# stateless-consensus/phant

Measured on AMD Instinct MI355X. Metric: mpt_proofs_verified_per_sec_depth8, higher is better.
Workload: dtype u64; 1 GPU; config3: 100000 synthetic depth-8 account proofs per GPU against one state root (7 x 532 B full branches + 112 B leaf, 3868 B and 29 Keccak-f per proof, 1% corrupted/exclusion, no cross-proof dedup); every launch sequence in flight verifies its own witness (seeds 2..3: distinct data per slot), 30 back-to-back passes per timed step; parallelism=key-sharded x1, verify_mode=flat, streams=2

## Files before the change

### phant_amd/csrc/mpt_verify_v3.hip

```cpp
#include <phant_platform.h>

#include "launch.h"
#include "mpt_verify_one.hip.h"
#include "coop_sponge.hip.h"
#include "verify_hash.hip.h"

namespace phant {
namespace v3 {
using namespace vh;

constexpr uint32_t HDR_PFN_BROKEN = 9;
constexpr uint32_t HDR_SLOW = 10;
constexpr uint32_t HDR_OPENED = 11;
constexpr uint32_t HDR_PARITY = 15;
constexpr uint32_t HDR_STAT = 1024;
constexpr uint32_t HDR_STAT_STRIPES = 16;
constexpr uint32_t HDR_STAT_WORDS = HDR_STAT_STRIPES * N_CLASS;
constexpr uint32_t HDR_STAT_END = HDR_STAT + 2u * HDR_STAT_WORDS;
constexpr uint32_t HDR_CUR = 256;
constexpr uint32_t HDR_WORDS = 768;
constexpr size_t HEADER_BYTES = 8192;
static_assert(HDR_STAT_END <= VERIFY_HEADER_WORDS && 4u * VERIFY_HEADER_WORDS <= HEADER_BYTES,
              "capi.hip copies VERIFY_HEADER_WORDS words back for the statistics");

PHANT_DEV uint32_t cursor_word(uint32_t cls, uint32_t stripe) { return HDR_CUR + 32u * stripe + cls; }



PHANT_DEV uint64_t key_prefix64(const uint8_t* __restrict__ key, uint32_t key_len) {
    uint64_t kb = 0;
    const uint32_t take = key_len < 8u ? key_len : 8u;
    for (uint32_t t = 0; t < take; ++t) kb |= (uint64_t)key[t] << (56u - 8u * t);
    return kb;
}
PHANT_DEV uint64_t key_prefix64_wide(const uint8_t* __restrict__ key, uint32_t key_len) {
    if (key_len < 8u) return key_prefix64(key, key_len);
    struct __attribute__((packed, aligned(1))) U64u { unsigned long long v; };
    return __builtin_bswap64(reinterpret_cast<const U64u*>(key)->v);
}
PHANT_DEV bool same_prefix(uint64_t x, uint64_t y, uint32_t d) { return d == 0u || ((x ^ y) >> (64u - 4u * d)) == 0ull; }
PHANT_DEV uint64_t group_hash(uint64_t kb, uint32_t root, uint32_t d) {
    const uint64_t pre = d ? (kb >> (64u - 4u * d)) : 0ull;
    uint64_t h = pre ^ ((uint64_t)(d + 1u) << 58) ^ ((uint64_t)root * 0x9E3779B97F4A7C15ull);
    h ^= h >> 33;
    h *= 0xff51afd7ed558ccdull;
    h ^= h >> 33;
    h *= 0xc4ceb9fe1a85ec53ull;
    h ^= h >> 33;
    return h;
}
PHANT_DEV uint32_t direct_index(uint64_t kb, uint32_t root, uint32_t d, uint32_t n_roots) {
    uint32_t width = 1u, below = 0u;
    for (uint32_t t = 0; t < d; ++t) {
        below += width;
        width <<= 4;
    }
    const uint32_t pre = d ? (uint32_t)(kb >> (64u - 4u * d)) : 0u;
    return n_roots * below + root * width + pre;
}
PHANT_DEV uint32_t slot_a(uint64_t h, uint32_t mask) { return (uint32_t)h & mask; }
PHANT_DEV uint32_t slot_b(uint64_t h, uint32_t mask) { return (uint32_t)(h >> 24) & mask; }

struct Args {
    VerifyArgs v;
    uint32_t total_nodes;
    uint32_t shallow;
    uint32_t direct;
    uint32_t* dtab;
    uint64_t* table;
    uint32_t tmask;
    uint32_t* rep;
    uint2* ent;
    uint32_t stripe_cap;
    uint32_t* hdr;
    uint32_t* digest;
    uint8_t* nstat;
};

PHANT_DEV void beside_the_hashing() { __builtin_amdgcn_s_setprio(3); }

__global__ void __launch_bounds__(256) zero_kernel(uint4* p, size_t n16, uint32_t* fail_count, uint32_t n_roots) {
    beside_the_hashing();
    const size_t i = (size_t)blockIdx.x * 256u + threadIdx.x;
    if (i < n16) p[i] = make_uint4(0u, 0u, 0u, 0u);
    if (fail_count)
        for (size_t r = i; r < n_roots; r += (size_t)gridDim.x * 256u) fail_count[r] = 0u;
}

struct ShallowLane {
    uint32_t p, d, j, root, len;
    uint64_t kb;
    bool act;
    bool valid;
    bool group;
    bool broken;
};
PHANT_DEV ShallowLane shallow_node(const Args& a, uint32_t p, uint32_t d) {
    ShallowLane L;
    L.p = p;
    L.d = d;
    L.j = 0;
    L.root = 0;
    L.len = 0;
    L.kb = 0;
    L.act = L.valid = L.group = L.broken = false;
    if (L.p >= a.v.n) return L;
    const uint32_t first = a.v.proof_first_node[L.p], last = a.v.proof_first_node[L.p + 1];
    if (last < first) {
        L.broken = L.d == 0u;
        return L;
    }
    if (last > a.total_nodes) return L;
    const uint32_t nn = 2u * a.v.key_len, cnt = last - first;
    const uint32_t end = cnt <= nn ? cnt : nn + 1u;
    if (L.d >= end) return L;
    L.act = true;
    L.j = first + L.d;
    L.root = a.v.root_idx ? a.v.root_idx[L.p] : 0u;
    const uint64_t e = a.v.node_off[L.j + 1], b = a.v.node_off[L.j];
    if (e >= b && e <= a.v.nodes_len && e - b <= 0x7fffffffull) {
        L.valid = true;
        L.len = (uint32_t)(e - b);
    }
    L.group = L.valid && L.len >= RATE && L.root < a.v.n_roots;
    if (L.group) L.kb = key_prefix64(a.v.keys + (uint64_t)a.v.key_len * L.p, a.v.key_len);
    return L;
}
PHANT_DEV ShallowLane shallow_lane(const Args& a, uint32_t g) {
    const uint32_t p = g / a.shallow;
    return shallow_node(a, p, g - p * a.shallow);
}

PHANT_DEV void clear_launch_state(const Args& a, uint32_t g, size_t lanes) {
    const uint32_t other = HDR_STAT + HDR_STAT_WORDS * ((a.hdr[HDR_PARITY] & 1u) ^ 1u);
    for (size_t i = g; i < HDR_WORDS + HDR_STAT_WORDS; i += lanes) {
        if (i < HDR_WORDS) {
            if (i != HDR_PARITY) a.hdr[i] = 0u;
        } else {
            a.hdr[other + (i - HDR_WORDS)] = 0u;
        }
    }
    if (a.v.fail_count)
        for (size_t r = g; r < a.v.n_roots; r += lanes) a.v.fail_count[r] = 0u;
}

__global__ void __launch_bounds__(256) propose_kernel(const Args a) {
    beside_the_hashing();
    const uint32_t g = blockIdx.x * 256u + threadIdx.x;
    clear_launch_state(a, g, (size_t)gridDim.x * 256u);
    const ShallowLane L = shallow_lane(a, g);
    if (L.act) a.nstat[L.j] = 0u;
    if (!L.group) return;
    if (L.d < a.direct) {
        a.dtab[direct_index(L.kb, L.root, L.d, a.v.n_roots)] = L.j + 1u;
    } else {
        const uint64_t h = group_hash(L.kb, L.root, L.d);
        const uint64_t entry = ((uint64_t)L.p << 32) | (uint64_t)(L.j + 1u);
        a.table[slot_a(h, a.tmask)] = entry;
        a.table[slot_b(h, a.tmask)] = entry;
    }
}

PHANT_DEV bool entry_matches(const Args& a, uint64_t en, const ShallowLane& L, uint32_t& node) {
    const uint32_t pr = (uint32_t)(en >> 32), j1 = (uint32_t)en;
    if (j1 == 0u || pr >= a.v.n) return false;
    node = j1 - 1u;
    if (pr == L.p) return node == L.j;
    const uint32_t f = a.v.proof_first_node[pr], l = a.v.proof_first_node[pr + 1];
    if (l < f || l > a.total_nodes || node < f || node >= l || node - f != L.d) return false;
    if ((a.v.root_idx ? a.v.root_idx[pr] : 0u) != L.root) return false;
    return same_prefix(key_prefix64(a.v.keys + (uint64_t)a.v.key_len * pr, a.v.key_len), L.kb, L.d);
}

PHANT_DEV uint64_t ent_index(const Args& a, uint32_t cls, uint32_t stripe, uint32_t at) {
    return ((uint64_t)cls * STRIPES + stripe) * a.stripe_cap + at;
}

PHANT_DEV bool wave_bytes_equal(const uint8_t* x, const uint8_t* y, uint32_t len, uint32_t lane) {
    uint32_t diff = 0;
    const uint32_t full = len & ~15u;
    for (uint32_t o = 16u * lane; o < full; o += 1024u) {
        const uint4 p = load16u(x + o), q = load16u(y + o);
        diff |= (p.x ^ q.x) | (p.y ^ q.y) | (p.z ^ q.z) | (p.w ^ q.w);
    }
    if (lane < (len & 15u)) diff |= (uint32_t)(x[full + lane] ^ y[full + lane]);
    return __ballot(diff != 0) == 0ull;
}

constexpr int COMPARE_UNROLL = 4;

__global__ void __launch_bounds__(256) PHANT_NUM_VGPR(48) dedup_kernel(const Args a) {
    constexpr uint32_t WAVES = 4;
    __shared__ uint32_t s_cnt[WAVES][N_LIST];
    __shared__ uint32_t s_base[N_LIST];
    beside_the_hashing();
    const uint32_t tid = threadIdx.x, lane = tid & 63u, wave = tid >> 6;
    const uint32_t NT = a.total_nodes;
    if (tid < WAVES * N_LIST) (&s_cnt[0][0])[tid] = 0u;
    const ShallowLane L = shallow_lane(a, blockIdx.x * 256u + tid);
    if (L.broken) a.hdr[HDR_PFN_BROKEN] = 1u;

    const uint32_t j = L.j;
    uint32_t cand = j;
    uint64_t b = 0, cb = 0;
    if (L.group) {
        uint32_t c = j;
        if (L.d < a.direct) {
            const uint32_t t = a.dtab[direct_index(L.kb, L.root, L.d, a.v.n_roots)];
            if (t) c = t - 1u;
        } else {
            const uint64_t h = group_hash(L.kb, L.root, L.d);
            uint32_t node;
            if (entry_matches(a, a.table[slot_a(h, a.tmask)], L, node)) c = node;
            else if (entry_matches(a, a.table[slot_b(h, a.tmask)], L, node)) c = node;
        }
        if (c != j && c < NT) {
            const uint64_t c0 = a.v.node_off[c], c1 = a.v.node_off[c + 1];
            if (c1 >= c0 && c1 <= a.v.nodes_len && c1 - c0 == L.len) {
                cand = c;
                cb = c0;
                b = a.v.node_off[j];
            }
        }
    }

    const uint32_t coff = 16u * (lane & 31u);
    const bool upper = lane >= 32u;
    const uint32_t b_lo = (uint32_t)b, b_hi = (uint32_t)(b >> 32), cb_lo = (uint32_t)cb, cb_hi = (uint32_t)(cb >> 32);
    bool differs = false;
    const bool is532 = cand != j && L.len == BRANCH_LEN;
    unsigned long long todo = __ballot(is532);
    while (todo) {
        uint32_t i0[COMPARE_UNROLL], i1[COMPARE_UNROLL];
        uint4 x[COMPARE_UNROLL], y[COMPARE_UNROLL];
        uint32_t i = 0;
#pragma unroll
        for (int u = 0; u < COMPARE_UNROLL; ++u) {
            if (todo) {
                i = (uint32_t)__builtin_ctzll(todo);
                todo &= todo - 1ull;
            }
            i0[u] = i;
            if (todo) {
                i = (uint32_t)__builtin_ctzll(todo);
                todo &= todo - 1ull;
            }
            i1[u] = i;
            const uint64_t own0 = lane_u64(b_lo, b_hi, i0[u]), own1 = lane_u64(b_lo, b_hi, i1[u]);
            const uint64_t oth0 = lane_u64(cb_lo, cb_hi, i0[u]), oth1 = lane_u64(cb_lo, cb_hi, i1[u]);
            x[u] = load16u(a.v.nodes + (upper ? own1 : own0) + coff);
            y[u] = load16u(a.v.nodes + (upper ? oth1 : oth0) + coff);
        }
#pragma unroll
        for (int u = 0; u < COMPARE_UNROLL; ++u) {
            uint32_t diff = x[u].x ^ y[u].x;
            diff = __builtin_amdgcn_bitop3_b32(x[u].y, y[u].y, diff, 0xBE);
            diff = __builtin_amdgcn_bitop3_b32(x[u].z, y[u].z, diff, 0xBE);
            diff = __builtin_amdgcn_bitop3_b32(x[u].w, y[u].w, diff, 0xBE);
            const unsigned long long m = __ballot(diff != 0);
            if ((uint32_t)m != 0u && lane == i0[u]) differs = true;
            if ((uint32_t)(m >> 32) != 0u && lane == i1[u]) differs = true;
        }
    }
    if (is532 && !differs) {
        const uint8_t* const own = a.v.nodes + b + (BRANCH_LEN - 28u);
        const uint8_t* const oth = a.v.nodes + cb + (BRANCH_LEN - 28u);
        const uint4 p0 = load16u(own), p1 = load16u(own + 12), q0 = load16u(oth), q1 = load16u(oth + 12);
        uint32_t diff = (p0.x ^ q0.x) | (p0.y ^ q0.y) | (p0.z ^ q0.z) | (p0.w ^ q0.w);
        diff |= (p1.x ^ q1.x) | (p1.y ^ q1.y) | (p1.z ^ q1.z) | (p1.w ^ q1.w);
        if (diff) differs = true;
    }
    todo = __ballot(cand != j && L.len != BRANCH_LEN);
    while (todo) {
        const uint32_t i = (uint32_t)__builtin_ctzll(todo);
        todo &= todo - 1ull;
        const uint32_t ll = lane_u32(L.len, i);
        const bool eq = wave_bytes_equal(a.v.nodes + lane_u64(b_lo, b_hi, i), a.v.nodes + lane_u64(cb_lo, cb_hi, i), ll, lane);
        if (lane == i && !eq) differs = true;
    }
    if (differs) cand = j;
    if (L.act) a.rep[j] = cand;

    const uint32_t cls = (L.act && L.valid && cand == j) ? node_list(L.len) : CLASS_NONE;
    uint32_t my_rank = 0;
    __syncthreads();
    todo = __ballot(cls != CLASS_NONE);
    while (todo) {
        const uint32_t c0 = lane_u32(cls, (uint32_t)__builtin_ctzll(todo));
        const unsigned long long m = __ballot(cls == c0);
        if (lane == 0) s_cnt[wave][c0] = (uint32_t)__popcll(m);
        if (cls == c0) my_rank = (uint32_t)__popcll(m & ((1ull << lane) - 1ull));
        todo &= ~m;
    }
    __syncthreads();
    const uint32_t stripe = blockIdx.x % STRIPES;
    if (tid < N_LIST) {
        uint32_t tot = 0;
        for (uint32_t w = 0; w < WAVES; ++w) tot += s_cnt[w][tid];
        s_base[tid] = tot ? atomicAdd(&a.hdr[cursor_word(tid, stripe)], tot) : 0u;
    }
    __syncthreads();
    if (cls != CLASS_NONE) {
        uint32_t at = s_base[cls] + my_rank;
        for (uint32_t w = 0; w < wave; ++w) at += s_cnt[w][cls];
        a.ent[ent_index(a, cls, stripe, at)] = make_uint2(j, L.p);
    }
}


PHANT_DEV const uint8_t* ref_location(const Args& a, uint32_t j, uint32_t d, uint32_t root, uint32_t nib_parent, uint64_t b) {
    if (d == 0u) return root < a.v.n_roots ? a.v.roots + 32ull * root : nullptr;
    if (nib_parent >= 16u) return nullptr;
    const uint64_t pb = a.v.node_off[j - 1u];
    if (pb > b || b - pb != BRANCH_LEN) return nullptr;
    return a.v.nodes + pb + (4u + 33u * nib_parent);
}

struct RefBytes { uint4 lo, hi; };
PHANT_DEV RefBytes load_ref(const uint8_t* q) {
    RefBytes r;
    r.lo = r.hi = make_uint4(0, 0, 0, 0);
    if (q) {
        r.lo = load16u(q);
        r.hi = load16u(q + 16);
    }
    return r;
}
PHANT_DEV bool digest_equals(const Sponge& s, const RefBytes& r) {
    const uint32_t diff = (s.lo[0] ^ r.lo.x) | (s.hi[0] ^ r.lo.y) | (s.lo[1] ^ r.lo.z) | (s.hi[1] ^ r.lo.w) |
                          (s.lo[2] ^ r.hi.x) | (s.hi[2] ^ r.hi.y) | (s.lo[3] ^ r.hi.z) | (s.hi[3] ^ r.hi.w);
    return diff == 0u;
}
PHANT_DEV void store_node_digest(const Args& a, uint32_t j, const Sponge& s) {
    uint4* o = reinterpret_cast<uint4*>(a.digest + 8ull * j);
    o[0] = make_uint4(s.lo[0], s.hi[0], s.lo[1], s.hi[1]);
    o[1] = make_uint4(s.lo[2], s.hi[2], s.lo[3], s.hi[3]);
}


PHANT_DEV bool list_role(const Args& a, uint32_t q, const uint32_t lane) {
    static_assert(N_QUEUE > 64u && N_QUEUE <= 128u, "two lists per lane");
    const uint32_t cnt_a = a.hdr[cursor_word(queue_class(lane), lane % STRIPES)];
    const uint32_t cnt_b = lane + 64u < N_QUEUE ? a.hdr[cursor_word(queue_class(lane + 64u), (lane + 64u) % STRIPES)] : 0u;
    const uint32_t ch_a = (cnt_a + 63u) / 64u, ch_b = (cnt_b + 63u) / 64u;
    const uint32_t incl_a = wave_inclusive_scan(ch_a, lane);
    uint32_t li, before, cnt;
    const unsigned long long m_a = __ballot(q < incl_a);
    if (m_a) {
        const uint32_t l = (uint32_t)__builtin_ctzll(m_a);
        li = l;
        before = lane_u32(incl_a, l) - lane_u32(ch_a, l);
        cnt = lane_u32(cnt_a, l);
    } else {
        const uint32_t incl_b = lane_u32(incl_a, 63u) + wave_inclusive_scan(ch_b, lane);
        const unsigned long long m_b = __ballot(q < incl_b);
        if (!m_b) return false;
        const uint32_t l = (uint32_t)__builtin_ctzll(m_b);
        li = l + 64u;
        before = lane_u32(incl_b, l) - lane_u32(ch_b, l);
        cnt = lane_u32(cnt_b, l);
    }
    const uint32_t cls = queue_class(li), stripe = li % STRIPES;
    uint32_t idx = (q - before) * 64u + lane;
    idx = idx < cnt ? idx : cnt - 1u;
    const uint2 en = a.ent[ent_index(a, cls, stripe, idx)];
    const uint32_t j = en.x;
    const uint8_t* const safe_end = a.v.nodes + a.v.nodes_len;
    const uint64_t b = a.v.node_off[j];
    const uint32_t len = (uint32_t)(a.v.node_off[j + 1] - b);
    const uint8_t* const p = a.v.nodes + b;

    const uint8_t* refp = nullptr;
    {
        const uint32_t owner = en.y;
        const uint32_t d = j - a.v.proof_first_node[owner];
        const uint32_t root = a.v.root_idx ? a.v.root_idx[owner] : 0u;
        uint32_t nibp = 16u;
        if (d >= 1u && d - 1u < 2u * a.v.key_len) nibp = key_nibble(a.v.keys + (uint64_t)a.v.key_len * owner, d - 1u);
        refp = ref_location(a, j, d, root, nibp, b);
    }
    const RefBytes ref = load_ref(refp);

    Sponge s;
    uint32_t bad;
    const uint32_t len0 = (uint32_t)__builtin_amdgcn_readfirstlane(len);
    if (cls == LIST_B532) {
        bad = hash_b532<true>(s, p);
    } else if (cls == 0u && __ballot(len != len0 || p + RATE > safe_end) == 0ull) {
        hash_short_uniform(s, p, len0);
        bad = 1u;
    } else {
        hash_any(s, p, len, safe_end);
        bad = 1u;
    }
    uint32_t ns = NS_HASHED | (bad == 0u ? NS_CANON : 0u);
    if (refp) ns |= NS_LINK_CHECKED | (digest_equals(s, ref) ? NS_LINK_OK : 0u);
    a.nstat[j] = (uint8_t)ns;
    store_node_digest(a, j, s);
    return true;
}

constexpr uint32_t DEEP_LEVELS = 8;

template <bool SOLO>
PHANT_DEV void deep_role(const Args& a, const uint32_t w, const uint32_t lane, const uint32_t waves_per_level, const uint32_t levels,
                         uint32_t (&s_ref)[8][256]) {
    const uint32_t level = w / waves_per_level;
    if (level >= levels) return;
    const uint32_t p = (w % waves_per_level) * 64u + lane;
    const uint8_t* const safe_end = a.v.nodes + a.v.nodes_len;
    const uint32_t nn = 2u * a.v.key_len;
    uint32_t hashed[N_CLASS] = {0, 0, 0, 0, 0, 0, 0, 0};
    const uint32_t stat_buf = a.hdr[HDR_PARITY] & 1u;
    for (uint32_t d = a.shallow + level;; d += levels) {
        uint32_t first = 0, count = 0, root = 0;
        if (p < a.v.n) {
            first = a.v.proof_first_node[p];
            const uint32_t last = a.v.proof_first_node[p + 1];
            if (last >= first && last <= a.total_nodes) count = last - first;
            if constexpr (SOLO) {
                if (last < first) a.hdr[HDR_PFN_BROKEN] = 1u;
            }
            if (a.v.root_idx) root = a.v.root_idx[p];
        }
        if (__ballot(d < count) == 0ull) break;
        const uint32_t j = first + d;
        bool active = d < count;
        uint64_t b = 0;
        uint32_t len = 0;
        if (active) {
            const uint64_t e = a.v.node_off[j + 1];
            b = a.v.node_off[j];
            active = e >= b && e <= a.v.nodes_len && e - b <= 0x7fffffffull;
            len = active ? (uint32_t)(e - b) : 0u;
            if (!active) a.nstat[j] = 0u;
        }
        const bool roomy = a.v.nodes_len >= BRANCH_LEN;
        const uint8_t* const ptr = a.v.nodes + (active ? b : 0ull);
        const uint8_t* refp = nullptr;
        if (active) {
            const uint8_t* const key = a.v.keys + (uint64_t)a.v.key_len * p;
            const uint32_t nibp = (d >= 1u && d - 1u < nn) ? key_nibble(key, d - 1u) : 16u;
            refp = ref_location(a, j, d, root, nibp, b);
        }
        {
            const RefBytes ref = load_ref(refp);
            const uint32_t t = threadIdx.x;
            s_ref[0][t] = ref.lo.x; s_ref[1][t] = ref.lo.y; s_ref[2][t] = ref.lo.z; s_ref[3][t] = ref.lo.w;
            s_ref[4][t] = ref.hi.x; s_ref[5][t] = ref.hi.y; s_ref[6][t] = ref.hi.z; s_ref[7][t] = ref.hi.w;
        }
        {
            const uint32_t cls = len / RATE < N_CLASS ? len / RATE : N_CLASS - 1u;
#pragma unroll
            for (uint32_t c = 0; c < N_CLASS; ++c) hashed[c] += (uint32_t)__popcll(__ballot(active && cls == c));
        }
        enum : uint32_t { F_ACTIVE = 1u, F_REF = 2u, F_CANON = 4u };
        uint32_t flags = (active ? F_ACTIVE : 0u) | (refp != nullptr ? F_REF : 0u);
        Sponge s;
        const bool is532 = active && len == BRANCH_LEN;
        if (roomy && __ballot(is532) != 0ull) {
            const uint32_t bad = hash_b532<true>(s, is532 ? ptr : a.v.nodes);
            if (is532 && bad == 0u) flags |= F_CANON;
        }
        const bool rest = active && !(roomy && is532);
        if (__ballot(rest) != 0ull) {
            const uint32_t len0 = (uint32_t)__builtin_amdgcn_readfirstlane(len);
            if (len0 < RATE && __ballot(!rest || len != len0 || ptr + RATE > safe_end) == 0ull) {
                hash_short_uniform(s, ptr, len0);
            } else if (rest) {
                hash_any(s, ptr, len, safe_end);
            }
        }
        if (flags & F_ACTIVE) {
            const uint32_t j = a.v.proof_first_node[p] + d;
            uint32_t ns = NS_HASHED | ((flags & F_CANON) ? NS_CANON : 0u);
            if (flags & F_REF) {
                const uint32_t t = threadIdx.x;
                RefBytes ref;
                ref.lo = make_uint4(s_ref[0][t], s_ref[1][t], s_ref[2][t], s_ref[3][t]);
                ref.hi = make_uint4(s_ref[4][t], s_ref[5][t], s_ref[6][t], s_ref[7][t]);
                ns |= NS_LINK_CHECKED | (digest_equals(s, ref) ? NS_LINK_OK : 0u);
            }
            a.nstat[j] = (uint8_t)ns;
            store_node_digest(a, j, s);
        }
    }
    if (lane < N_CLASS) {
        uint32_t mine = 0;
#pragma unroll
        for (uint32_t c = 0; c < N_CLASS; ++c) mine = lane == c ? hashed[c] : mine;
        if (mine) atomicAdd(&a.hdr[HDR_STAT + HDR_STAT_WORDS * stat_buf + N_CLASS * (w % HDR_STAT_STRIPES) + lane], mine);
    }
}

template <bool SOLO>
__global__ void __launch_bounds__(256, 4) hash_deep_kernel(const Args a, const uint32_t waves_per_level, const uint32_t levels) {
    __shared__ uint32_t s_ref[8][256];
    const uint32_t w = (uint32_t)__builtin_amdgcn_readfirstlane(blockIdx.x * 4u + (threadIdx.x >> 6));
    deep_role<SOLO>(a, w, threadIdx.x & 63u, waves_per_level, levels, s_ref);
}
constexpr uint32_t COOP_MAX_NODES = 2048;
constexpr uint32_t WAVE_MAX_NODES = 2048;
constexpr uint32_t NO_STAT = 0xffffffffu;
PHANT_DEV void coop_node(const Args& a, const CoopLane& c, const uint32_t l, const uint32_t base, const bool present, const uint32_t p,
                         const uint32_t j, const uint32_t d, const uint32_t root, const uint32_t stat_word) {
    struct __attribute__((packed, aligned(1))) U64 { unsigned long long v; };
    const uint32_t nn = 2u * a.v.key_len;
    bool active = false;
    uint32_t len = 0;
    uint64_t b = 0;
    if (present) {
        const uint64_t e = a.v.node_off[j + 1];
        b = a.v.node_off[j];
        active = e >= b && e <= a.v.nodes_len && e - b <= 0x7fffffffull;
        len = active ? (uint32_t)(e - b) : 0u;
        if (!active && l == 0) a.nstat[j] = 0u;
    }
    const uint8_t* const ptr = a.v.nodes + (active ? b : 0ull);
    const uint8_t* refp = nullptr;
    if (active) {
        const uint8_t* const key = a.v.keys + (uint64_t)a.v.key_len * p;
        refp = ref_location(a, j, d, root, (d >= 1u && d - 1u < nn) ? key_nibble(key, d - 1u) : 16u, b);
    }
    const uint32_t nb = active ? len / RATE + 1u : 0u;
    const uint32_t nb_other = __shfl(nb, (int)(base ^ 32u), 64);
    const uint32_t nb_max = nb > nb_other ? nb : nb_other;
    const bool branch = active && len == BRANCH_LEN;
    uint32_t lo = 0, hi = 0, dlo = 0, dhi = 0, bad = 0;
    for (uint32_t k = 0; k < nb_max; ++k) {
        if (k < nb && l < 17u) {
            const uint32_t off = k * RATE + 8u * l;
            unsigned long long w = 0;
            if (off + 8u <= len) {
                w = reinterpret_cast<const U64*>(ptr + off)->v;
            } else {
#pragma unroll
                for (uint32_t t = 0; t < 8u; ++t) {
                    const uint32_t q = off + t;
                    if (q < len) w |= (unsigned long long)ptr[q] << (8u * t);
                    else if (q == len) w |= 0x01ull << (8u * t);
                }
            }
            if (k + 1u == nb && l == 16u) w |= 0x80ull << 56;
            if (branch) {
#pragma unroll
                for (uint32_t t = 0; t < 8u; ++t) {
                    const uint32_t q = off + t;
                    const uint32_t byte = (uint32_t)(w >> (8u * t)) & 0xffu;
                    const int want = q == 0u ? 0xf9 : q == 1u ? 0x02 : q == 2u ? 0x11 : q == BRANCH_LEN - 1u ? 0x80 : (q < BRANCH_LEN && (q - 3u) % 33u == 0u) ? 0xa0 : -1;
                    if (want >= 0 && byte != (uint32_t)want) bad = 1u;
                }
            }
            lo ^= (uint32_t)w;
            hi ^= (uint32_t)(w >> 32);
        }
        coop_permute(c, lo, hi);
        if (k + 1u == nb) {
            dlo = lo;
            dhi = hi;
        }
    }
    bool ne = false;
    if (refp && l < 4u) {
        const unsigned long long r = reinterpret_cast<const U64*>(refp + 8u * l)->v;
        ne = (uint32_t)r != dlo || (uint32_t)(r >> 32) != dhi;
    }
    const uint32_t any_bad = (uint32_t)(__ballot(bad != 0u) >> base), any_ne = (uint32_t)(__ballot(ne) >> base);
    if (active) {
        uint32_t ns = NS_HASHED | ((branch && any_bad == 0u) ? NS_CANON : 0u);
        if (refp) ns |= NS_LINK_CHECKED | (any_ne == 0u ? NS_LINK_OK : 0u);
        if (l < 4u) {
            a.digest[8ull * j + 2u * l] = dlo;
            a.digest[8ull * j + 2u * l + 1u] = dhi;
        }
        if (l == 0) {
            a.nstat[j] = (uint8_t)ns;
            const uint32_t cls = len / RATE < N_CLASS ? len / RATE : N_CLASS - 1u;
            if (stat_word != NO_STAT) atomicAdd(&a.hdr[stat_word + cls], 1u);
        }
    }
}

__global__ void __launch_bounds__(256) hash_coop_kernel(const Args a, const uint32_t levels) {
    const uint32_t tid = threadIdx.x, l = tid & 31u, base = tid & 32u;
    const uint32_t h = blockIdx.x * (blockDim.x >> 5) + (tid >> 5);
    const uint32_t p = h / levels, level = h % levels;
    uint32_t first = 0, count = 0, root = 0;
    if (p < a.v.n) {
        first = a.v.proof_first_node[p];
        const uint32_t last = a.v.proof_first_node[p + 1];
        if (last >= first && last <= a.total_nodes) count = last - first;
        if (last < first && l == 0) a.hdr[HDR_PFN_BROKEN] = 1u;
        if (a.v.root_idx) root = a.v.root_idx[p];
    }
    const uint32_t stat_word = HDR_STAT + HDR_STAT_WORDS * (a.hdr[HDR_PARITY] & 1u) + N_CLASS * (h % HDR_STAT_STRIPES);
    const CoopLane c = coop_lane(l, base, gridDim.x * (blockDim.x >> 6) <= 1024u);
    for (uint32_t d = level;; d += levels) {
        if (__ballot(d < count) == 0ull) break;
        coop_node(a, c, l, base, d < count, p, first + d, d, root, stat_word);
    }
}

PHANT_DEV void wave_node(const Args& a, const WaveLane& c, const uint32_t l, const uint32_t p, const uint32_t j, const uint32_t d, const uint32_t root,
                         const uint32_t stat_word) {
    struct __attribute__((packed, aligned(1))) U64 { unsigned long long v; };
    const uint32_t nn = 2u * a.v.key_len;
    const uint64_t e = a.v.node_off[j + 1], b = a.v.node_off[j];
    const bool active = e >= b && e <= a.v.nodes_len && e - b <= 0x7fffffffull;
    if (!active) {
        if (l == 0) a.nstat[j] = 0u;
        return;
    }
    const uint32_t len = (uint32_t)(e - b);
    const uint8_t* const ptr = a.v.nodes + b;
    const uint8_t* const key = a.v.keys + (uint64_t)a.v.key_len * p;
    const uint8_t* const refp = ref_location(a, j, d, root, (d >= 1u && d - 1u < nn) ? key_nibble(key, d - 1u) : 16u, b);
    const uint32_t nb = len / RATE + 1u;
    const bool branch = len == BRANCH_LEN;
    uint32_t lo = 0, hi = 0, bad = 0;
    for (uint32_t k = 0; k < nb; ++k) {
        if (c.word < 17u) {
            const uint32_t off = k * RATE + 8u * c.word;
            unsigned long long w = 0;
            if (off + 8u <= len) {
                w = reinterpret_cast<const U64*>(ptr + off)->v;
            } else {
#pragma unroll
                for (uint32_t t = 0; t < 8u; ++t) {
                    const uint32_t q = off + t;
                    if (q < len) w |= (unsigned long long)ptr[q] << (8u * t);
                    else if (q == len) w |= 0x01ull << (8u * t);
                }
            }
            if (k + 1u == nb && c.word == 16u) w |= 0x80ull << 56;
            if (branch) {
#pragma unroll
                for (uint32_t t = 0; t < 8u; ++t) {
                    const uint32_t q = off + t;
                    const uint32_t byte = (uint32_t)(w >> (8u * t)) & 0xffu;
                    const int want = q == 0u ? 0xf9 : q == 1u ? 0x02 : q == 2u ? 0x11 : q == BRANCH_LEN - 1u ? 0x80 : (q < BRANCH_LEN && (q - 3u) % 33u == 0u) ? 0xa0 : -1;
                    if (want >= 0 && byte != (uint32_t)want) bad = 1u;
                }
            }
            lo ^= (uint32_t)w;
            hi ^= (uint32_t)(w >> 32);
        }
        wave_permute(c, lo, hi);
    }
    bool ne = false;
    if (refp && l < 4u) {
        const unsigned long long r = reinterpret_cast<const U64*>(refp + 8u * l)->v;
        ne = (uint32_t)r != lo || (uint32_t)(r >> 32) != hi;
    }
    const bool any_bad = __ballot(bad != 0u) != 0ull, any_ne = __ballot(ne) != 0ull;
    uint32_t ns = NS_HASHED | ((branch && !any_bad) ? NS_CANON : 0u);
    if (refp) ns |= NS_LINK_CHECKED | (!any_ne ? NS_LINK_OK : 0u);
    if (l < 4u) {
        a.digest[8ull * j + 2u * l] = lo;
        a.digest[8ull * j + 2u * l + 1u] = hi;
    }
    if (l == 0) {
        a.nstat[j] = (uint8_t)ns;
        const uint32_t cls = len / RATE < N_CLASS ? len / RATE : N_CLASS - 1u;
        if (stat_word != NO_STAT) atomicAdd(&a.hdr[stat_word + cls], 1u);
    }
}

__global__ void __launch_bounds__(256) hash_wave_kernel(const Args a, const uint32_t levels) {
    const uint32_t tid = threadIdx.x, l = tid & 63u;
    const uint32_t h = blockIdx.x * (blockDim.x >> 6) + (tid >> 6);
    const uint32_t p = h / levels, level = h % levels;
    if (p >= a.v.n) return;
    const uint32_t first = a.v.proof_first_node[p], last = a.v.proof_first_node[p + 1];
    uint32_t count = 0;
    if (last >= first && last <= a.total_nodes) count = last - first;
    if (last < first && l == 0) a.hdr[HDR_PFN_BROKEN] = 1u;
    const uint32_t root = a.v.root_idx ? a.v.root_idx[p] : 0u;
    const uint32_t stat_word = HDR_STAT + HDR_STAT_WORDS * (a.hdr[HDR_PARITY] & 1u) + N_CLASS * (h % HDR_STAT_STRIPES);
    const WaveLane c = wave_lane(l);
    for (uint32_t d = level; d < count; d += levels) wave_node(a, c, l, p, first + d, d, root, stat_word);
}

__global__ void __launch_bounds__(256, 4) hash_list_kernel(const Args a) {
    __builtin_amdgcn_s_setprio(2);
    const uint32_t q = (uint32_t)__builtin_amdgcn_readfirstlane(blockIdx.x * 4u + (threadIdx.x >> 6));
    (void)list_role(a, q, threadIdx.x & 63u);
}

enum : uint32_t { LINK_GENERIC = 0, LINK_FAST = 1, LINK_HASH_OK = 2, LINK_BAD_HASH = 3 };

PHANT_DEV uint32_t code_of(uint32_t ns, bool has_nibble) {
    if (!(ns & NS_HASHED) || !(ns & NS_LINK_CHECKED)) return LINK_GENERIC;
    if (!(ns & NS_LINK_OK)) return LINK_BAD_HASH;
    return (has_nibble && (ns & NS_CANON)) ? LINK_FAST : LINK_HASH_OK;
}


template <bool DIRECT>
__global__ void __launch_bounds__(256) walk_kernel(const Args a) {
    __shared__ uint32_t s_stage[256 * WALK_SLOT_DW];
    beside_the_hashing();
    const uint32_t i = blockIdx.x * 256u + threadIdx.x;
    const bool in = i < a.v.n;
    uint32_t status = PHANT_PROOF_PRESENT;
    uint32_t r = 0;
    if (in) {
        uint32_t* const slot = s_stage + threadIdx.x * WALK_SLOT_DW;
        const uint8_t* const slot_node = reinterpret_cast<const uint8_t*>(slot);
        const uint8_t* const nodes_end = a.v.nodes + a.v.nodes_len;
        uint64_t voff = 0;
        uint32_t vlen = 0;
        const uint32_t first = a.v.proof_first_node[i], last = a.v.proof_first_node[i + 1];
        r = a.v.root_idx ? a.v.root_idx[i] : 0u;
        if (last < first || last > a.total_nodes || r >= a.v.n_roots) {
            status = PHANT_PROOF_BAD_INPUT;
        } else if (last == first) {
            uint32_t rw[8];
            GlobalBytes rb{a.v.roots + 32ull * r};
#pragma unroll
            for (int k = 0; k < 8; ++k) rw[k] = rb.u32(4 * k);
            status = is_empty_root(rw) ? PHANT_PROOF_ABSENT : PHANT_PROOF_INVALID_EMPTY;
        } else if (a.hdr[HDR_PFN_BROKEN] != 0u) {
            status = STATUS_NEEDS_SLOW;
        } else {
            const uint8_t* const key = a.v.keys + (uint64_t)a.v.key_len * i;
            const uint32_t nn = 2u * a.v.key_len;
            uint32_t sx = 0;
            if constexpr (!DIRECT) {
                const uint32_t cnt = last - first, end = cnt <= nn ? cnt : nn + 1u;
                sx = end < a.shallow ? end : a.shallow;
            }
            const uint8_t* const slot_key = reinterpret_cast<const uint8_t*>(slot + WALK_STAGE_BYTES / 4);
            const bool key_in_lds = a.v.key_len <= WALK_KEY_BYTES;
            if (key_in_lds) {
                uint8_t* kdst = reinterpret_cast<uint8_t*>(slot + WALK_STAGE_BYTES / 4);
                for (uint32_t t = 0; t < a.v.key_len; ++t) kdst[t] = key[t];
            }
            WalkState w;
            w.pos = 0;
            w.status = PHANT_PROOF_BAD_INPUT;
            w.value_pay = w.value_len = w.ref_pay = w.ref_total = 0;
            uint32_t used = first;
            status = 0xffffffffu;

            bool hash_known = false;
            uint32_t rprev = 0;
            for (bool run = true; run && used < last;) {
                const uint32_t base = used, dbase = used - first;
                const uint8_t* lp = a.nstat + base;
                const uint32_t c0 = load4u(lp), c1 = load4u(lp + 4);
                uint32_t rj[8], nsr[8], rpar[8];
                if constexpr (!DIRECT) {
                    if (dbase < sx) {
                        const uint8_t* rp = reinterpret_cast<const uint8_t*>(a.rep + base);
                        const uint4 r0 = load16u(rp), r1 = load16u(rp + 16);
                        rj[0] = r0.x; rj[1] = r0.y; rj[2] = r0.z; rj[3] = r0.w;
                        rj[4] = r1.x; rj[5] = r1.y; rj[6] = r1.z; rj[7] = r1.w;
#pragma unroll
                        for (int u = 0; u < 8; ++u) {
                            const bool sh = dbase + u < sx && base + u < last && rj[u] < a.total_nodes;
                            rj[u] = sh ? rj[u] : base + u;
                        }
#pragma unroll
                        for (int u = 0; u < 8; ++u) {
                            const bool copy = rj[u] != base + u;
                            nsr[u] = copy ? a.nstat[rj[u]] : 0u;
                            rpar[u] = (copy && rj[u] >= 1u && dbase + u >= 1u) ? a.rep[rj[u] - 1u] : 0xffffffffu;
                        }
                    } else {
#pragma unroll
                        for (int u = 0; u < 8; ++u) {
                            rj[u] = base + u;
                            nsr[u] = 0u;
                            rpar[u] = 0xffffffffu;
                        }
                    }
                }
#pragma unroll
                for (int u = 0; u < 8; ++u) {
                    if (!run || used >= last) continue;
                    const uint32_t own = ((u < 4 ? c0 : c1) >> (8 * (u & 3))) & 0xffu;
                    uint32_t c, me = used;
                    if constexpr (DIRECT) {
                        c = code_of(own, w.pos < nn);
                    } else {
                        me = rj[u];
                        if (me == used) c = code_of(own, w.pos < nn);
                        else if (used == first || rpar[u] == rprev) c = code_of(nsr[u], w.pos < nn);
                        else if (!(nsr[u] & NS_HASHED)) c = LINK_GENERIC;
                        else {
                            const uint8_t* rb = a.v.nodes + a.v.node_off[used - 1u] + (4u + 33u * key_nibble(key, w.pos - 1u));
                            const uint4 w0 = load16u(rb), w1 = load16u(rb + 16);
                            const uint4* dg = reinterpret_cast<const uint4*>(a.digest + 8ull * me);
                            const uint4 d0 = dg[0], d1 = dg[1];
                            const uint32_t diff = (d0.x ^ w0.x) | (d0.y ^ w0.y) | (d0.z ^ w0.z) | (d0.w ^ w0.w) |
                                                  (d1.x ^ w1.x) | (d1.y ^ w1.y) | (d1.z ^ w1.z) | (d1.w ^ w1.w);
                            c = diff ? LINK_BAD_HASH : ((w.pos < nn && (nsr[u] & NS_CANON)) ? LINK_FAST : LINK_HASH_OK);
                        }
                    }
                    if (c == LINK_FAST) {
                        ++used;
                        w.pos += 1;
                        rprev = me;
                    } else {
                        run = false;
                        if (c == LINK_BAD_HASH) status = PHANT_PROOF_BAD_HASH;
                        else hash_known = c == LINK_HASH_OK;
                    }
                }
            }

            uint32_t want[8] = {0, 0, 0, 0, 0, 0, 0, 0};
            if (status == 0xffffffffu && !hash_known) {
                if (used == first) {
                    GlobalBytes rb{a.v.roots + 32ull * r};
#pragma unroll
                    for (int k = 0; k < 8; ++k) want[k] = rb.u32(4 * k);
                } else {
                    const uint32_t nibp = key_nibble(key, w.pos - 1u);
                    const uint8_t* rb = a.v.nodes + a.v.node_off[used - 1u] + (4u + 33u * nibp);
                    const uint4 r0 = load16u(rb), r1 = load16u(rb + 16);
                    want[0] = r0.x; want[1] = r0.y; want[2] = r0.z; want[3] = r0.w;
                    want[4] = r1.x; want[5] = r1.y; want[6] = r1.z; want[7] = r1.w;
                }
            }
            bool by_hash = true;
            const uint8_t* cur = nullptr;
            uint32_t cur_len = 0, opened = 0;
            const uint8_t* staged_from = nullptr;
            for (;;) {
                if (status != 0xffffffffu) break;
                ++opened;
                if (by_hash) {
                    if (used == last) {
                        status = PHANT_PROOF_MISSING_NODE;
                        break;
                    }
                    const uint32_t j = used;
                    const uint64_t b = a.v.node_off[j], e = a.v.node_off[j + 1];
                    if (e < b || e > a.v.nodes_len || e - b > 0x7fffffffull) {
                        status = PHANT_PROOF_BAD_INPUT;
                        break;
                    }
                    cur = a.v.nodes + b;
                    cur_len = (uint32_t)(e - b);
                    ++used;
                    if (hash_known) {
                        hash_known = false;
                    } else {
                        uint32_t rj = j;
                        if constexpr (!DIRECT) {
                            if (j - first < sx) rj = a.rep[j];
                        }
                        if (!(rj < a.total_nodes && (a.nstat[rj] & NS_HASHED))) {
                            status = STATUS_NEEDS_SLOW;
                            break;
                        }
                        const uint4* dg = reinterpret_cast<const uint4*>(a.digest + 8ull * rj);
                        const uint4 d0 = dg[0], d1 = dg[1];
                        const uint32_t diff = (d0.x ^ want[0]) | (d0.y ^ want[1]) | (d0.z ^ want[2]) | (d0.w ^ want[3]) |
                                              (d1.x ^ want[4]) | (d1.y ^ want[5]) | (d1.z ^ want[6]) | (d1.w ^ want[7]);
                        if (diff) {
                            status = PHANT_PROOF_BAD_HASH;
                            break;
                        }
                        if ((a.nstat[rj] & NS_CANON) && w.pos < nn) {
                            const uint8_t* rb = cur + (4u + 33u * key_nibble(key, w.pos));
                            const uint4 r0 = load16u(rb), r1 = load16u(rb + 16);
                            want[0] = r0.x; want[1] = r0.y; want[2] = r0.z; want[3] = r0.w;
                            want[4] = r1.x; want[5] = r1.y; want[6] = r1.z; want[7] = r1.w;
                            w.pos += 1;
                            continue;
                        }
                    }
                    staged_from = nullptr;
                    const uint32_t padded = (cur_len + 15u) & ~15u;
                    if (cur_len <= WALK_STAGE_BYTES && cur + padded <= nodes_end) {
                        for (uint32_t o = 0; o < padded; o += 16u) {
                            const uint4 q = load16u(cur + o);
                            slot[o / 4u] = q.x;
                            slot[o / 4u + 1u] = q.y;
                            slot[o / 4u + 2u] = q.z;
                            slot[o / 4u + 3u] = q.w;
                        }
                        staged_from = cur;
                    }
                }
                auto step_from = [&](const uint8_t* nb, const uint8_t* kp) __attribute__((always_inline)) -> uint32_t {
                    GlobalBytes nd{nb};
                    const uint32_t st = walk_node(nd, cur_len, kp, nn, w);
                    if (st == STEP_HASH) {
#pragma unroll
                        for (int k = 0; k < 8; ++k) want[k] = nd.u32(w.ref_pay + 4 * k);
                    }
                    return st;
                };
                uint32_t step;
                if (!key_in_lds) step = step_from(cur, key);
                else if (staged_from) step = step_from(slot_node + (cur - staged_from), slot_key);
                else step = step_from(cur, slot_key);
                if (step == STEP_DONE) break;
                if (step == STEP_HASH) {
                    by_hash = true;
                } else {
                    cur = cur + w.ref_pay;
                    cur_len = w.ref_total;
                    by_hash = false;
                }
            }
            if (opened > 1u) atomicAdd(&a.hdr[HDR_OPENED], opened);
            if (status == 0xffffffffu) {
                status = w.status;
                if (status == PHANT_PROOF_PRESENT || status == PHANT_PROOF_ABSENT) {
                    if (used != last) {
                        status = PHANT_PROOF_EXTRA_NODES;
                    } else if (status == PHANT_PROOF_PRESENT) {
                        voff = (uint64_t)(cur - a.v.nodes) + w.value_pay;
                        vlen = w.value_len;
                    }
                }
            }
        }
        if (status == STATUS_NEEDS_SLOW) {
            atomicAdd(&a.hdr[HDR_SLOW], 1u);
            status = verify_one(a.v, i, voff, vlen);
        }
        a.v.status[i] = (uint8_t)status;
        if (a.v.value_off) a.v.value_off[i] = voff;
        if (a.v.value_len) a.v.value_len[i] = vlen;
    }
    if (blockIdx.x == 0 && threadIdx.x == 0) a.hdr[HDR_PARITY] ^= 1u;
    if (a.v.fail_count) {
        const bool bad = in && !(status == PHANT_PROOF_PRESENT || status == PHANT_PROOF_ABSENT);
        if (a.v.root_idx == nullptr || a.v.n_roots == 1) {
            const unsigned long long m = __ballot(bad);
            if ((threadIdx.x & 63u) == 0 && m) atomicAdd(&a.v.fail_count[0], (uint32_t)__popcll(m));
        } else if (bad) {
            atomicAdd(&a.v.fail_count[r < a.v.n_roots ? r : 0u], 1u);
        }
    }
}

__global__ void __launch_bounds__(256) stream_read_kernel(const uint4* __restrict__ p, size_t n16, uint32_t* sink, size_t mask) {
    const size_t stride = (size_t)gridDim.x * 256u;
    size_t i = (size_t)blockIdx.x * 256u + threadIdx.x;
    uint4 acc = make_uint4(0u, 0u, 0u, 0u);
    for (; i + 7u * stride < n16; i += 8u * stride) {
        uint4 v[8];
#pragma unroll
        for (int u = 0; u < 8; ++u) v[u] = p[(i + (size_t)u * stride) & mask];
#pragma unroll
        for (int u = 0; u < 8; ++u) {
            acc.x ^= v[u].x;
            acc.y ^= v[u].y;
            acc.z ^= v[u].z;
            acc.w ^= v[u].w;
        }
    }
    for (; i < n16; i += stride) {
        const uint4 v = p[i & mask];
        acc.x ^= v.x;
        acc.y ^= v.y;
        acc.z ^= v.z;
        acc.w ^= v.w;
    }
    const uint32_t x = acc.x ^ acc.y ^ acc.z ^ acc.w;
    if (x == 0x9e3779b9u && sink) sink[blockIdx.x & 255u] = x;
}

static size_t rnd256(size_t x) { return (x + 255) / 256 * 256; }

constexpr uint64_t HASH_EVERYTHING_BELOW_BYTES = 72000000ull;

static uint32_t shallow_levels(uint32_t n, uint32_t n_roots, uint64_t nodes_len, int32_t forced) {
    if (forced >= 0) return (uint32_t)forced < MAX_SHALLOW ? (uint32_t)forced : MAX_SHALLOW;
    if (n < 2 || nodes_len < HASH_EVERYTHING_BELOW_BYTES) return 0;
    uint64_t n_eff = n;
    if (n_roots > 1u) {
        uint64_t r = 1;
        while ((r + 1) * (r + 1) <= n_roots) ++r;
        n_eff = n / r ? n / r : 1;
    }
    uint32_t s = 1;
    uint64_t groups = 16;
    while (s < MAX_SHALLOW && groups <= 4ull * n_eff) {
        ++s;
        groups *= 16;
    }
    return s;
}

constexpr uint64_t DIRECT_MAX_ENTRIES = 1ull << 21;
static uint32_t direct_levels(uint32_t n_roots, uint32_t shallow, uint64_t& entries) {
    uint32_t d = 0;
    uint64_t below = 0, width = 1;
    entries = 0;
    while (d < shallow && (below + width) * n_roots <= DIRECT_MAX_ENTRIES) {
        below += width;
        width *= 16;
        ++d;
        entries = below * n_roots;
    }
    return d;
}

static uint32_t table_entries(uint32_t n, uint32_t n_roots, uint32_t direct, uint32_t shallow, uint32_t total_nodes) {
    uint64_t per_root = 0, g = 1;
    for (uint32_t d = 0; d < shallow && per_root < (1ull << 40); ++d, g *= 16)
        if (d >= direct) per_root += g;
    uint64_t groups = per_root * (n_roots ? n_roots : 1u);
    const uint64_t by_nodes = (uint64_t)n * (shallow - direct) < total_nodes ? (uint64_t)n * (shallow - direct) : total_nodes;
    if (groups > by_nodes) groups = by_nodes;
    uint32_t t = 1024;
    while (t < 4 * groups && t < (1u << 26)) t <<= 1;
    return t;
}

struct Layout {
    size_t nstat, dtab, table, rep, ent, digest, end;
    uint32_t stripe_cap;
};
static Layout layout(uint32_t total_nodes, uint32_t te, uint64_t direct_entries, uint64_t lanes) {
    const size_t tn = total_nodes;
    Layout l;
    const uint64_t wgs = (lanes + 255u) / 256u;
    l.stripe_cap = (uint32_t)((wgs + STRIPES - 1u) / STRIPES * 256u);
    size_t p = HEADER_BYTES;
    l.nstat = p;  p += rnd256(tn + 16);
    l.dtab = p;   p += rnd256((size_t)direct_entries * 4);
    l.table = p;  p += rnd256((size_t)te * 8);
    l.rep = p;    p += rnd256(tn * 4 + 64);
    l.ent = p;    p += rnd256((size_t)N_LIST * STRIPES * l.stripe_cap * 8u);
    l.digest = p; p += rnd256(tn * 32);
    l.end = p + 1024;
    return l;
}

size_t workspace_bytes(uint32_t total_nodes) {
    uint32_t t = 1024;
    while (t < 4ull * total_nodes && t < (1u << 26)) t <<= 1;
    const uint64_t lanes = (uint64_t)total_nodes + 256u * STRIPES;
    return layout(total_nodes, t, DIRECT_MAX_ENTRIES, lanes).end;
}

static void bind(Args& a, uint8_t* ws, const Layout& l, uint32_t te) {
    a.hdr = reinterpret_cast<uint32_t*>(ws);
    a.nstat = ws + l.nstat;
    a.dtab = reinterpret_cast<uint32_t*>(ws + l.dtab);
    a.table = reinterpret_cast<uint64_t*>(ws + l.table);
    a.tmask = te - 1u;
    a.rep = reinterpret_cast<uint32_t*>(ws + l.rep);
    a.ent = reinterpret_cast<uint2*>(ws + l.ent);
    a.stripe_cap = l.stripe_cap;
    a.digest = reinterpret_cast<uint32_t*>(ws + l.digest);
}

}

size_t verify_workspace_bytes(uint32_t total_nodes) { return v3::workspace_bytes(total_nodes); }

hipError_t launch_mpt_verify(const VerifyArgs& v_in, uint32_t total_nodes, uint8_t* ws, int32_t dedup_levels,
                                hipStream_t st, const FlatSide* side, const VerifyTune& tune) {
    using namespace v3;
    VerifyArgs v = v_in;
    v.total_nodes = total_nodes;
    if (v.n == 0) return hipSuccess;
    Args a;
    a.v = v;
    a.total_nodes = total_nodes;
    a.shallow = shallow_levels(v.n, v.n_roots, v.nodes_len, dedup_levels);
    while (a.shallow && (uint64_t)v.n * a.shallow > (uint64_t)total_nodes + 256u * STRIPES) --a.shallow;
    if (tune.last_shallow) *tune.last_shallow = total_nodes ? a.shallow : 0u;
    uint64_t direct_entries = 0;
    a.direct = direct_levels(v.n_roots, a.shallow, direct_entries);
    const uint32_t te = table_entries(v.n, v.n_roots, a.direct, a.shallow, total_nodes);
    const uint64_t lanes = (uint64_t)v.n * a.shallow;
    const Layout l = layout(total_nodes, te, direct_entries, lanes);
    bind(a, ws, l, te);
    hipError_t e = hipSuccess;
    const uint32_t pg = (v.n + 255u) / 256u;
    const uint32_t wpl = (v.n + 63u) / 64u;
    const uint64_t avg_len = total_nodes ? (total_nodes + v.n - 1u) / v.n : 0u;
    const uint32_t deep_levels = avg_len + 1u <= a.shallow ? 1u
                                 : (uint32_t)(avg_len + 1u - a.shallow < DEEP_LEVELS ? avg_len + 1u - a.shallow : DEEP_LEVELS);
    const uint32_t deep_wgs = (wpl * deep_levels + 3u) / 4u;
    if (tune.last_form) *tune.last_form = (a.shallow == 0u || total_nodes == 0u) ? 0u : 1u;
    if (a.shallow == 0u || total_nodes == 0u) {
        a.shallow = 0;
        const size_t zero_n16 = l.dtab / 16;
        hipLaunchKernelGGL(zero_kernel, dim3((uint32_t)((zero_n16 + 255) / 256)), dim3(256), 0, st, reinterpret_cast<uint4*>(ws),
                           zero_n16, v.fail_count, v.n_roots);
        const uint64_t halves = (uint64_t)v.n * deep_levels;
        if (total_nodes && total_nodes <= tune.coop_max && !tune.no_coop && halves <= 4ull * COOP_MAX_NODES)
            if (halves <= WAVE_MAX_NODES && !tune.no_wave) {
                if (halves <= 512u) hipLaunchKernelGGL(hash_wave_kernel, dim3((uint32_t)halves), dim3(64), 0, st, a, deep_levels);
                else hipLaunchKernelGGL(hash_wave_kernel, dim3((uint32_t)((halves + 3u) / 4u)), dim3(256), 0, st, a, deep_levels);
            } else if (halves <= 1024u) {
                hipLaunchKernelGGL(hash_coop_kernel, dim3((uint32_t)((halves + 1u) / 2u)), dim3(64), 0, st, a, deep_levels);
            } else {
                hipLaunchKernelGGL(hash_coop_kernel, dim3((uint32_t)((halves + 7u) / 8u)), dim3(256), 0, st, a, deep_levels);
            }
        else if (total_nodes)
            hipLaunchKernelGGL(hash_deep_kernel<true>, dim3(deep_wgs), dim3(256), 0, st, a, wpl, deep_levels);
        hipLaunchKernelGGL(walk_kernel<true>, dim3(pg), dim3(256), 0, st, a);
        return hipGetLastError();
    }
    const uint32_t sg = (uint32_t)((lanes + 255u) / 256u);
    const bool two = side && side->stream && side->fork && side->join && !tune.serial;
    hipStream_t hs = two ? side->stream : st;
    const uint64_t listed = lanes < total_nodes ? lanes : total_nodes;
    const uint32_t list_wgs = (uint32_t)((listed + 255u) / 256u) + (N_QUEUE + 3u) / 4u;
    const uint32_t hash_lds = two ? tune.hash_lds : 0u;
    if (two) {
        if ((e = hipEventRecord(side->fork, st)) != hipSuccess) return e;
        if ((e = hipStreamWaitEvent(side->stream, side->fork, 0)) != hipSuccess) return e;
    }
    hipEvent_t* const kev = (!two && tune.serial) ? tune.kernel_ev : nullptr;
    auto mark = [&](int i) {
        if (kev && e == hipSuccess) e = hipEventRecord(kev[i], st);
    };
    if (tune.diag) {
        const bool three = two && side->stream2 && side->join2;
        hipStream_t h2 = three ? side->stream2 : st;
        if (two) {
            if ((e = hipEventRecord(side->fork, st)) != hipSuccess) return e;
            if ((e = hipStreamWaitEvent(side->stream, side->fork, 0)) != hipSuccess) return e;
            if (three && (e = hipStreamWaitEvent(side->stream2, side->fork, 0)) != hipSuccess) return e;
        }
        if (tune.diag & 1u) {
            const uint32_t lds = tune.diag == 3u ? hash_lds : 0u;
            hipLaunchKernelGGL(hash_deep_kernel<false>, dim3(deep_wgs), dim3(256), lds, hs, a, wpl, deep_levels);
            hipLaunchKernelGGL(hash_list_kernel, dim3(list_wgs), dim3(256), lds ? lds + 8192u : 0u, st, a);
        }
        if (tune.diag & 2u) {
            const uint32_t wgs = tune.diag_stream_wgs ? tune.diag_stream_wgs : 2048u;
            size_t mask = ~(size_t)0;
            if (tune.diag_stream_mb) {
                size_t r16 = (size_t)tune.diag_stream_mb << 16;
                while (r16 > v.nodes_len / 16u) r16 >>= 1;
                mask = r16 ? r16 - 1u : 0u;
            }
            hipLaunchKernelGGL(stream_read_kernel, dim3(wgs), dim3(256), 0, h2, reinterpret_cast<const uint4*>(v.nodes),
                               (size_t)(v.nodes_len / 16u), tune.diag_sink, mask);
        }
        if (two) {
            if ((e = hipEventRecord(side->join, side->stream)) != hipSuccess) return e;
            if ((e = hipStreamWaitEvent(st, side->join, 0)) != hipSuccess) return e;
            if (three) {
                if ((e = hipEventRecord(side->join2, side->stream2)) != hipSuccess) return e;
                if ((e = hipStreamWaitEvent(st, side->join2, 0)) != hipSuccess) return e;
            }
        }
        return hipGetLastError();
    }
    mark(0);
    hipLaunchKernelGGL(propose_kernel, dim3(sg), dim3(256), 0, st, a);
    mark(1);
    hipLaunchKernelGGL(hash_deep_kernel<false>, dim3(deep_wgs), dim3(256), hash_lds, hs, a, wpl, deep_levels);
    mark(2);
    if (two && (e = hipEventRecord(side->join, side->stream)) != hipSuccess) return e;
    hipLaunchKernelGGL(dedup_kernel, dim3(sg), dim3(256), 0, st, a);
    mark(3);
    hipLaunchKernelGGL(hash_list_kernel, dim3(list_wgs), dim3(256), hash_lds ? hash_lds + 8192u : 0u, st, a);
    mark(4);
    if (two && (e = hipStreamWaitEvent(st, side->join, 0)) != hipSuccess) return e;
    hipLaunchKernelGGL(walk_kernel<false>, dim3(pg), dim3(256), 0, st, a);
    mark(5);
    if (e != hipSuccess) return e;
    return hipGetLastError();
}

void verify_stats_from_header(const uint32_t* hdr, uint32_t hashed[8]) {
    using namespace v3;
    uint32_t lists[N_LIST];
    for (uint32_t c = 0; c < N_LIST; ++c) {
        lists[c] = 0;
        for (uint32_t s = 0; s < STRIPES; ++s) lists[c] += hdr[HDR_CUR + 32u * s + c];
    }
    const uint32_t buf = (hdr[HDR_PARITY] & 1u) ^ 1u;
    for (uint32_t c = 0; c < N_CLASS; ++c) {
        hashed[c] = lists[c];
        for (uint32_t s = 0; s < HDR_STAT_STRIPES; ++s) hashed[c] += hdr[HDR_STAT + HDR_STAT_WORDS * buf + N_CLASS * s + c];
    }
    hashed[BRANCH_LEN / RATE] += lists[LIST_B532];
}
void verify_tier_stats_from_header(const uint32_t* hdr, uint32_t out[4]) {
    using namespace v3;
    out[0] = out[1] = out[2] = out[3] = 0;
    for (uint32_t c = 0; c < N_LIST; ++c) {
        uint32_t cnt = 0;
        for (uint32_t s = 0; s < STRIPES; ++s) cnt += hdr[HDR_CUR + 32u * s + c];
        out[0] += cnt;
        out[1] += cnt * (c == LIST_B532 ? BRANCH_LEN / RATE + 1u : c + 1u);
    }
    const uint32_t buf = (hdr[HDR_PARITY] & 1u) ^ 1u;
    for (uint32_t c = 0; c < N_CLASS; ++c)
        for (uint32_t s = 0; s < HDR_STAT_STRIPES; ++s) {
            const uint32_t cnt = hdr[HDR_STAT + HDR_STAT_WORDS * buf + N_CLASS * s + c];
            out[2] += cnt;
            out[3] += cnt * (c + 1u);
        }
}
void verify_paths_from_header(const uint32_t* hdr, uint32_t out[2]) {
    out[0] = hdr[v3::HDR_SLOW];
    out[1] = hdr[v3::HDR_OPENED];
}

}
```

Measured before the change: 540.3 million proofs/s.

## Skip digest stores for link-verified nodes and bound list kernel by chunk count

Hash kernels no longer write the 32-byte node digest when the node's hash already matched its parent reference. The walk kernel instead reads the expected bytes straight from the parent branch (or root) for such nodes. The last dedup block also computes the total list chunk count so surplus hash_list waves exit early. This trades digest write traffic and idle waves for an extra last-block fence/atomic and extra address logic in the walk, and it depends on ref_location being valid for every link-OK node.

```diff
diff --git a/phant_amd/csrc/mpt_verify_v3.hip b/phant_amd/csrc/mpt_verify_v3.hip
--- a/phant_amd/csrc/mpt_verify_v3.hip
+++ b/phant_amd/csrc/mpt_verify_v3.hip
@@ -12,6 +12,8 @@
 constexpr uint32_t HDR_PFN_BROKEN = 9;
 constexpr uint32_t HDR_SLOW = 10;
 constexpr uint32_t HDR_OPENED = 11;
+constexpr uint32_t HDR_DEDUP_LEFT = 12;
+constexpr uint32_t HDR_CHUNKS = 13;
 constexpr uint32_t HDR_PARITY = 15;
 constexpr uint32_t HDR_STAT = 1024;
 constexpr uint32_t HDR_STAT_STRIPES = 16;
@@ -193,6 +195,7 @@
     constexpr uint32_t WAVES = 4;
     __shared__ uint32_t s_cnt[WAVES][N_LIST];
     __shared__ uint32_t s_base[N_LIST];
+    __shared__ uint32_t s_last;
     beside_the_hashing();
     const uint32_t tid = threadIdx.x, lane = tid & 63u, wave = tid >> 6;
     const uint32_t NT = a.total_nodes;
@@ -305,6 +308,20 @@
         for (uint32_t w = 0; w < wave; ++w) at += s_cnt[w][cls];
         a.ent[ent_index(a, cls, stripe, at)] = make_uint2(j, L.p);
     }
+    if (tid == 0) {
+        __threadfence();
+        s_last = atomicAdd(&a.hdr[HDR_DEDUP_LEFT], 1u) == gridDim.x - 1u ? 1u : 0u;
+    }
+    __syncthreads();
+    if (!s_last || wave != 0u) return;
+    __threadfence();
+    static_assert(N_QUEUE > 64u && N_QUEUE <= 128u, "two lists per lane");
+    const uint32_t cnt_a = __hip_atomic_load(&a.hdr[cursor_word(queue_class(lane), lane % STRIPES)], __ATOMIC_RELAXED, __HIP_MEMORY_SCOPE_AGENT);
+    const uint32_t cnt_b = lane + 64u < N_QUEUE ? __hip_atomic_load(&a.hdr[cursor_word(queue_class(lane + 64u), (lane + 64u) % STRIPES)],
+                                                                       __ATOMIC_RELAXED, __HIP_MEMORY_SCOPE_AGENT)
+                                                  : 0u;
+    const uint32_t chunks = wave_inclusive_scan((cnt_a + 63u) / 64u + (cnt_b + 63u) / 64u, lane);
+    if (lane == 63u) a.hdr[HDR_CHUNKS] = chunks;
 }
 
 
@@ -472,7 +489,6 @@
             }
         }
         if (flags & F_ACTIVE) {
-            const uint32_t j = a.v.proof_first_node[p] + d;
             uint32_t ns = NS_HASHED | ((flags & F_CANON) ? NS_CANON : 0u);
             if (flags & F_REF) {
                 const uint32_t t = threadIdx.x;
@@ -482,7 +498,7 @@
                 ns |= NS_LINK_CHECKED | (digest_equals(s, ref) ? NS_LINK_OK : 0u);
             }
             a.nstat[j] = (uint8_t)ns;
-            store_node_digest(a, j, s);
+            if (!(ns & NS_LINK_OK)) store_node_digest(a, j, s);
         }
     }
     if (lane < N_CLASS) {
@@ -569,7 +585,7 @@
     if (active) {
         uint32_t ns = NS_HASHED | ((branch && any_bad == 0u) ? NS_CANON : 0u);
         if (refp) ns |= NS_LINK_CHECKED | (any_ne == 0u ? NS_LINK_OK : 0u);
-        if (l < 4u) {
+        if (l < 4u && !(ns & NS_LINK_OK)) {
             a.digest[8ull * j + 2u * l] = dlo;
             a.digest[8ull * j + 2u * l + 1u] = dhi;
         }
@@ -655,7 +671,7 @@
     const bool any_bad = __ballot(bad != 0u) != 0ull, any_ne = __ballot(ne) != 0ull;
     uint32_t ns = NS_HASHED | ((branch && !any_bad) ? NS_CANON : 0u);
     if (refp) ns |= NS_LINK_CHECKED | (!any_ne ? NS_LINK_OK : 0u);
-    if (l < 4u) {
+    if (l < 4u && !(ns & NS_LINK_OK)) {
         a.digest[8ull * j + 2u * l] = lo;
         a.digest[8ull * j + 2u * l + 1u] = hi;
     }
@@ -682,8 +698,9 @@
 }
 
 __global__ void __launch_bounds__(256, 4) hash_list_kernel(const Args a) {
+    const uint32_t q = (uint32_t)__builtin_amdgcn_readfirstlane(blockIdx.x * 4u + (threadIdx.x >> 6));
+    if (q >= a.hdr[HDR_CHUNKS]) return;
     __builtin_amdgcn_s_setprio(2);
-    const uint32_t q = (uint32_t)__builtin_amdgcn_readfirstlane(blockIdx.x * 4u + (threadIdx.x >> 6));
     (void)list_role(a, q, threadIdx.x & 63u);
 }
 
@@ -852,19 +869,28 @@
                         if constexpr (!DIRECT) {
                             if (j - first < sx) rj = a.rep[j];
                         }
-                        if (!(rj < a.total_nodes && (a.nstat[rj] & NS_HASHED))) {
+                        const uint32_t nsj = rj < a.total_nodes ? a.nstat[rj] : 0u;
+                        if (!(nsj & NS_HASHED)) {
                             status = STATUS_NEEDS_SLOW;
                             break;
                         }
-                        const uint4* dg = reinterpret_cast<const uint4*>(a.digest + 8ull * rj);
-                        const uint4 d0 = dg[0], d1 = dg[1];
+                        const uint8_t* dgp = reinterpret_cast<const uint8_t*>(a.digest + 8ull * rj);
+                        if ((DIRECT || j - first >= sx) && (nsj & NS_LINK_CHECKED) && (nsj & NS_LINK_OK)) {
+                            const uint32_t dj = j - first;
+                            dgp = ref_location(a, j, dj, r, (dj >= 1u && dj - 1u < nn) ? key_nibble(key, dj - 1u) : 16u, b);
+                            if (dgp == nullptr) {
+                                status = STATUS_NEEDS_SLOW;
+                                break;
+                            }
+                        }
+                        const uint4 d0 = load16u(dgp), d1 = load16u(dgp + 16);
                         const uint32_t diff = (d0.x ^ want[0]) | (d0.y ^ want[1]) | (d0.z ^ want[2]) | (d0.w ^ want[3]) |
                                               (d1.x ^ want[4]) | (d1.y ^ want[5]) | (d1.z ^ want[6]) | (d1.w ^ want[7]);
                         if (diff) {
                             status = PHANT_PROOF_BAD_HASH;
                             break;
                         }
-                        if ((a.nstat[rj] & NS_CANON) && w.pos < nn) {
+                        if ((nsj & NS_CANON) && w.pos < nn) {
                             const uint8_t* rb = cur + (4u + 33u * key_nibble(key, w.pos));
                             const uint4 r0 = load16u(rb), r1 = load16u(rb + 16);
                             want[0] = r0.x; want[1] = r0.y; want[2] = r0.z; want[3] = r0.w;
```

Result: slower. 385.2 million proofs/s (-28.7%).
